# jacobswan1/ViTCAP

Hardware: AMD Instinct MI355X
Metric: images/sec end-to-end greedy caption (20 tok), ViT-B/16-384 (higher is better)
Workload: dtype bf16; 1 GPU; BASELINE configs[1]: ViT-B/16-384 greedy decode (20 tok), batch 64 bf16 per GPU, seeded random-init weights, uniform(-1,1) 384x384 images resident in HBM; batch_per_gpu=64, global_batch=64, decode=greedy, max_length=20, parallelism=replicas x1 (no data-path collective), launch=2-slot batch pipeline (encode of step i+1 || decode of step i), eager launches, streams_per_gpu=2

## Files before the change

vitcap_amd/csrc/call_state.h:

```cpp
#pragma once
#include <hip/hip_runtime.h>
#include <stdint.h>

void vitcap_set_error(const char* fmt, ...);

extern thread_local const int32_t* vc_tls_live;
struct VcEosExtra { int32_t id[3]; };
extern thread_local VcEosExtra vc_tls_eos_extra;
extern thread_local bool vc_tls_walk_rev;
extern thread_local bool vc_tls_zigzag;
extern thread_local const uint32_t* vc_tls_drop_salt;
extern thread_local hipEvent_t vc_tls_kev_start, vc_tls_kev_stop;
extern thread_local bool vc_tls_kev_used;
```

vitcap_amd/csrc/decode.hip:

```cpp
#include "common.h"
#include "rng.h"

namespace {

struct ArgMax {
  float v;
  int i;
};
__device__ __forceinline__ ArgMax am_better(ArgMax a, ArgMax b) {
  return (b.v > a.v || (b.v == a.v && b.i < a.i)) ? b : a;
}
__device__ __forceinline__ ArgMax wave_argmax(ArgMax a) {
#pragma unroll
  for (int o = 32; o > 0; o >>= 1) {
    ArgMax b;
    b.v = __shfl_xor(a.v, o, 64);
    b.i = __shfl_xor(a.i, o, 64);
    a = am_better(a, b);
  }
  return a;
}

__global__ void greedy_init_kernel(int64_t* ids, int32_t* unf, float* sum_lp, float* cnt, int B, int max_len, int bos,
                                   int pad, int32_t* live) {
// ... 307 lines not shown
  if (lane == 0) { s_am[w] = best; s_second[w] = second; s_f[w] = bx; }
  __syncthreads();
  if (tid == 0) {
    ArgMax bb = s_am[0];
    float ss = s_second[0], xx = s_f[0];
    for (int k = 1; k < 16; ++k) {
      const ArgMax nb = am_better(bb, s_am[k]);
      ss = fmaxf(fmaxf(ss, s_second[k]), (nb.i == bb.i) ? s_am[k].v : bb.v);
      xx = (nb.i == bb.i) ? xx : s_f[k];
      bb = nb;
    }
    if (margin_out) margin_out[(size_t)b * max_len + t] = bb.v - ss;
    const float lp = xx - m - logf(z);
    const int u = unf[b];
    const int add = u ? bb.i : pad;
    float s = sum_lp[b] + lp * (float)u;
    float c = cnt[b] + (float)u;
    int nu = u * (vc_is_eos(add, eos, eos_x) ? 0 : 1);
    int64_t outtok = add;
    if (t == max_len - 1) {
      if (raw_last) raw_last[b] = add;
      if (nu) outtok = eos;
      logprob_out[b] = s / c;
    }
    ids[(size_t)b * max_len + t] = outtok;
    sum_lp[b] = s;
    cnt[b] = c;
    unf[b] = nu;
    if (live && u && !nu) atomicSub(live, 1);
  }
}

constexpr int TK_PER_THREAD = 32;
__device__ __forceinline__ unsigned long long tk_key(float f, int i);
__device__ __forceinline__ float tk_val(unsigned long long k);
__device__ __forceinline__ int tk_idx(unsigned long long k);
__device__ __forceinline__ unsigned long long wave_max_u64(unsigned long long a);
__global__ __launch_bounds__(1024) void sigmoid_topk_kernel(const float* __restrict__ logits, int ldl, int V, int k,
                                                            float thresh, int64_t* __restrict__ out_ids,
                                                            float* __restrict__ out_prob,
                                                            int64_t* __restrict__ out_len) {
  __shared__ unsigned long long s_wmax[2][16];
  const int b = blockIdx.x, tid = threadIdx.x, lane = tid & 63, w = tid >> 6;
  const float* row = logits + (size_t)b * ldl;
  unsigned long long key[TK_PER_THREAD];
  unsigned long long tmax = 0ull;
#pragma unroll
  for (int j = 0; j < TK_PER_THREAD; ++j) {
    const int i = tid + j * 1024;
    key[j] = i < V ? tk_key(1.0f / (1.0f + expf(-row[i])), i) : 0ull;
    tmax = key[j] > tmax ? key[j] : tmax;
  }
  int nlen = 0;
  for (int r = 0; r < k; ++r) {
    const unsigned long long wm = wave_max_u64(tmax);
    if (lane == 0) s_wmax[r & 1][w] = wm;
    __syncthreads();
    unsigned long long best = s_wmax[r & 1][0];
#pragma unroll
    for (int q = 1; q < 16; ++q) {
      const unsigned long long c = s_wmax[r & 1][q];
      best = c > best ? c : best;
    }
    if (tid == 0) {
      const float pv = tk_val(best);
      out_ids[(size_t)b * k + r] = tk_idx(best);
      out_prob[(size_t)b * k + r] = pv;
      if (pv >= thresh) ++nlen;
    }
    if (tmax == best) {
      tmax = 0ull;
#pragma unroll
      for (int j = 0; j < TK_PER_THREAD; ++j) {
        if (key[j] == best) key[j] = 0ull;
        tmax = key[j] > tmax ? key[j] : tmax;
      }
    }
  }
  if (tid == 0) out_len[b] = nlen;
}


__device__ __forceinline__ unsigned long long tk_key(float f, int i) {
  unsigned u = __float_as_uint(f);
  u = (u & 0x80000000u) ? ~u : (u | 0x80000000u);
  return ((unsigned long long)u << 32) | (unsigned)(~i);
}
__device__ __forceinline__ float tk_val(unsigned long long k) {
  unsigned u = (unsigned)(k >> 32);
  u = (u & 0x80000000u) ? (u & 0x7fffffffu) : ~u;
  return __uint_as_float(u);
}
__device__ __forceinline__ int tk_idx(unsigned long long k) { return (int)(~(unsigned)k); }
__device__ __forceinline__ unsigned long long wave_max_u64(unsigned long long a) {
#pragma unroll
  for (int o = 32; o > 0; o >>= 1) {
    const unsigned lo = __shfl_xor((unsigned)a, o, 64), hi = __shfl_xor((unsigned)(a >> 32), o, 64);
    const unsigned long long b = ((unsigned long long)hi << 32) | lo;
    a = b > a ? b : a;
  }
  return a;
}

__global__ __launch_bounds__(1024) void row_topk_lse_kernel(const float* __restrict__ logits, int ldl, int V, int k,
                                                            float* __restrict__ out_val, int* __restrict__ out_idx,
                                                            float* __restrict__ out_lse, const int32_t* __restrict__ live) {
  VC_LIVE_EXIT(live);
  constexpr int CAP = TK_PER_THREAD * 16;
  __shared__ unsigned long long s_cand[16][16];
  __shared__ unsigned long long s_list[CAP];
  __shared__ unsigned long long s_thr;
  __shared__ float s_sum[16];
// ... 400 lines not shown
  VC_REQUIRE(logits && ids && rows > 0 && V > 0 && ldl >= V && t >= 1 && t <= ld_ids && t <= 64 && penalty > 0.f,
             "repetition_penalty: bad arguments (t=%d, penalty=%g)", t, (double)penalty);
  hipLaunchKernelGGL(repetition_penalty_kernel, dim3((rows + 3) / 4), dim3(256), 0, (hipStream_t)stream, logits, ldl, V, ids,
                     ld_ids, t, penalty, rows, vc_tls_live);
  VC_LAUNCH_CHECK("repetition_penalty");
  return VITCAP_OK;
}

extern "C" int vitcap_greedy_init(int64_t* ids, int32_t* unfinished, float* sum_lp, float* cnt, int B, int max_len,
                                  int bos, int pad, void* stream) {
  VC_REQUIRE(ids && unfinished && sum_lp && cnt && B > 0 && max_len > 1, "greedy_init: bad arguments");
  const int n = B * max_len;
  hipLaunchKernelGGL(greedy_init_kernel, dim3((n + 255) / 256), dim3(256), 0, (hipStream_t)stream, ids, unfinished,
                     sum_lp, cnt, B, max_len, bos, pad, (int32_t*)vc_tls_live);
  VC_LAUNCH_CHECK("greedy_init");
  return VITCAP_OK;
}

extern "C" int vitcap_greedy_step(const float* logits, int ldl, int V, int64_t* ids, int32_t* unfinished,
                                  float* sum_lp, float* cnt, float* logprob_out, float* margin_out, int64_t* raw_last,
                                  int B, int t, int max_len, int eos, int pad, void* stream) {
  VC_REQUIRE(logits && ids && unfinished && sum_lp && cnt && logprob_out, "greedy_step: null pointer");
  VC_REQUIRE(B > 0 && V > 0 && ldl >= V && t >= 1 && t < max_len, "greedy_step: bad sizes (t=%d)", t);
  hipLaunchKernelGGL(greedy_step_kernel, dim3(B), dim3(1024), 0, (hipStream_t)stream, logits, ldl, V, ids, unfinished,
                     sum_lp, cnt, logprob_out, margin_out, raw_last, t, max_len, eos, pad, (int32_t*)vc_tls_live, vc_tls_eos_extra);
  VC_LAUNCH_CHECK("greedy_step");
  return VITCAP_OK;
}

extern "C" int vitcap_sigmoid_topk(const float* logits, int ldl, int V, int k, float thresh, int64_t* out_ids,
                                   float* out_prob, int64_t* out_len, int B, void* stream) {
  VC_REQUIRE(logits && out_ids && out_prob && out_len && B > 0, "sigmoid_topk: bad arguments");
  VC_REQUIRE(k >= 1 && k <= 64 && V <= TK_PER_THREAD * 1024 && ldl >= V, "sigmoid_topk: k=%d V=%d unsupported", k, V);
  hipLaunchKernelGGL(sigmoid_topk_kernel, dim3(B), dim3(1024), 0, (hipStream_t)stream, logits, ldl, V, k, thresh,
                     out_ids, out_prob, out_len);
  VC_LAUNCH_CHECK("sigmoid_topk");
  return VITCAP_OK;
}


extern "C" int vitcap_row_topk_lse(const float* logits, int ldl, int V, int k, float* out_val, int32_t* out_idx,
                                   float* out_lse, int rows, void* stream) {
  VC_REQUIRE(logits && out_val && out_idx && out_lse && rows > 0, "row_topk_lse: bad arguments");
  VC_REQUIRE(k >= 1 && k <= 16 && V <= TK_PER_THREAD * 1024 && ldl >= V, "row_topk_lse: k=%d V=%d unsupported", k, V);
  hipLaunchKernelGGL(row_topk_lse_kernel, dim3(rows), dim3(1024), 0, (hipStream_t)stream, logits, ldl, V, k, out_val,
                     out_idx, out_lse, vc_tls_live);
  VC_LAUNCH_CHECK("row_topk_lse");
  return VITCAP_OK;
}

extern "C" int vitcap_row_topk_pieces(const float* logits, int ldl, int V, const float* rowstat, int pieces, int k,
                                      float* out_val, int32_t* out_idx, float* out_lse, int rows, void* stream) {
  VC_REQUIRE(logits && rowstat && out_val && out_idx && out_lse && rows > 0, "row_topk_pieces: bad arguments");
  VC_REQUIRE(k >= 1 && k <= 16 && ldl >= V && pieces >= k && pieces <= 1024 && pieces * 32 >= V,
             "row_topk_pieces: k=%d V=%d pieces=%d unsupported", k, V, pieces);
  hipLaunchKernelGGL(row_topk_pieces_kernel, dim3(rows), dim3(256), 0, (hipStream_t)stream, logits, ldl, V, rowstat, pieces, k,
                     out_val, out_idx, out_lse, vc_tls_live);
  VC_LAUNCH_CHECK("row_topk_pieces");
  return VITCAP_OK;
}

static BeamState make_state(const vitcap_beam_state* s) {
  BeamState st;
  st.ids_in = s->ids_in; st.ids_out = s->ids_out; st.beam_scores = s->beam_scores; st.parent = s->parent;
  st.done = s->done; st.has_hyp = s->has_hyp; st.hyp_score = s->hyp_score; st.hyp_len = s->hyp_len;
  st.hyp_tok = s->hyp_tok;
  st.n_keep = s->n_keep;
  return st;
// ... 97 lines not shown
```

vitcap_amd/csrc/engine.cpp:

```cpp
#include <stdlib.h>
#include <string.h>

#include <new>
#include <utility>

#include "engine_internal.h"
#include "engine_layout.h"

using namespace vc;

namespace {

vitcap_gen_opts default_opts() {
  vitcap_gen_opts o;
  memset(&o, 0, sizeof(o));
  o.abi = VITCAP_ABI_VERSION;
  o.num_beams = 1;
  o.seqs_per_image = 1;
  o.num_keep_best = 1;
  o.max_length = VITCAP_MAXLEN;
  o.bos_token_id = 101; o.eos_token_id = 102; o.pad_token_id = 0; o.mask_token_id = 103;
  o.length_penalty = 1.0f;
  o.repetition_penalty = 1.0f;
  o.sampling.do_sample = 0; o.sampling.temperature = 1.0f; o.sampling.top_k = 0; o.sampling.top_p = 1.0f; o.sampling.seed = 0u;
// ... 50 lines not shown
    OPT_REQ(o.tag_visible == 0, "gen_opts: use_cbs with tag tokens visible to the caption is not built");
    OPT_REQ(o.max_length >= 3, "gen_opts: use_cbs needs max_length >= 3 (got %d)", o.max_length);
    OPT_REQ(o.cbs_no_repeat == 0 || o.cbs_no_repeat == 1, "gen_opts: cbs_no_repeat must be 0 or 1 (got %d)", o.cbs_no_repeat);
    for (int i = 0; i < 16; ++i)
      OPT_REQ(o.cbs_bad_ending[i] >= -1 && o.cbs_bad_ending[i] < VITCAP_VOCAB, "gen_opts: cbs_bad_ending[%d] = %d is neither -1 nor a token id", i, o.cbs_bad_ending[i]);
  }
#undef OPT_REQ
  return VITCAP_OK;
}

#define CK(call)             \
  do {                       \
    int rc_ = (call);        \
    if (rc_ != 0) return rc_; \
  } while (0)

#define HIPCK(call, what)                                                              \
  do {                                                                                 \
    hipError_t he_ = (call);                                                           \
    if (he_ != hipSuccess) {                                                           \
      vitcap_set_error("%s: %s", what, hipGetErrorString(he_));                        \
      return VITCAP_ELAUNCH;                                                           \
    }                                                                                  \
  } while (0)

void drop_graphs(vitcap_engine* e) {
  for (auto& g : e->graphs) {
    (void)hipGraphExecDestroy(g.exec);
    (void)hipGraphDestroy(g.graph);
  }
  e->graphs.clear();
}

enum { ROLE_SIDE = 0, ROLE_DEC2 = 1, ROLE_PART0 = 2 , ROLE_COUNT = 5 };
hipStream_t role_stream(int role) {
  static std::mutex mu;
  static hipStream_t pool[64][ROLE_COUNT] = {};
  int dev = 0;
  if (hipGetDevice(&dev) != hipSuccess || dev < 0 || dev >= 64 || role < 0 || role >= ROLE_COUNT) return nullptr;
  std::lock_guard<std::mutex> lk(mu);
  if (!pool[dev][role] && hipStreamCreateWithFlags(&pool[dev][role], hipStreamNonBlocking) != hipSuccess) pool[dev][role] = nullptr;
  return pool[dev][role];
}

int ensure_lane(int role, hipStream_t& st, hipEvent_t& ev_fork, hipEvent_t& ev_join, const char* what) {
  if (st) return VITCAP_OK;
  hipStream_t rs = role_stream(role);
  if (!rs || (!ev_fork && hipEventCreateWithFlags(&ev_fork, hipEventDisableTiming) != hipSuccess) ||
      (!ev_join && hipEventCreateWithFlags(&ev_join, hipEventDisableTiming) != hipSuccess)) {
    vitcap_set_error("%s stream creation failed", what);
    return VITCAP_ELAUNCH;
  }
  st = rs;
  return VITCAP_OK;
}
int ev_record(hipEvent_t ev, void* s, const char* what, const char* edge) {
  const hipError_t he = hipEventRecord(ev, (hipStream_t)s);
  if (he != hipSuccess) { vitcap_set_error("%s %s record: %s", what, edge, hipGetErrorString(he)); return VITCAP_ELAUNCH; }
  return VITCAP_OK;
}
int ev_wait(void* s, hipEvent_t ev, const char* what, const char* edge) {
  const hipError_t he = hipStreamWaitEvent((hipStream_t)s, ev, 0);
  if (he != hipSuccess) { vitcap_set_error("%s %s wait: %s", what, edge, hipGetErrorString(he)); return VITCAP_ELAUNCH; }
  return VITCAP_OK;
}
int fork(void* from, void* to, hipEvent_t ev, const char* what) {
  CK(ev_record(ev, from, what, "fork"));
// ... 119 lines not shown
                const vitcap_vit_block_w* next = nullptr) const {
    const int M = B * NV;
    if (!have_ln1) { CK(vitcap_layernorm_fwd(x_in, D, bw.n1_g, bw.n1_b, 1e-6f, h, nullptr, M, D, s)); zz(); }
    CK(gemm(h, D, bw.qkv_w, bw.qkv_b, nullptr, 0, qkv, 3 * D, M, 3 * D, D, VITCAP_ACT_NONE, VITCAP_OUT_BF16));
    zz();
    CK(vitcap_attn_dense_fwd(qkv, h, B, NV, 0.125f, s));
    zz();
    CK(gemm_ln(h, D, bw.proj_w, bw.proj_b, x_in, x, M, D, bw.n2_g, bw.n2_b, 1e-6f, h, nullptr));
    CK(gemm(h, D, bw.fc1_w, bw.fc1_b, nullptr, 0, mlp, 4 * D, M, 4 * D, D, VITCAP_ACT_GELU_ERF, VITCAP_OUT_BF16));
    zz();
    if (next) {
      CK(gemm_ln(mlp, 4 * D, bw.fc2_w, bw.fc2_b, x, x, M, 4 * D, next->n1_g, next->n1_b, 1e-6f, h, nullptr));
    } else {
      CK(gemm(mlp, 4 * D, bw.fc2_w, bw.fc2_b, x, D, x, D, M, D, 4 * D, VITCAP_ACT_NONE, VITCAP_OUT_F32));
      zz();
    }
    return VITCAP_OK;
  }

  int vit_block_cls_only(const vitcap_vit_block_w& bw, float* x, void* h, void* qkv, void* mlp, void* cls_h) const {
    const int M = B * NV;
    const int RS = NV * D;
    CK(gemm(h, D, (const char*)bw.qkv_w + (size_t)D * D * 2, bw.qkv_b + D, nullptr, 0, (char*)qkv + (size_t)D * 2, 3 * D, M, 2 * D, D,
            VITCAP_ACT_NONE, VITCAP_OUT_BF16));
    CK(gemm(h, RS, bw.qkv_w, bw.qkv_b, nullptr, 0, qkv, NV * 3 * D, B, D, D, VITCAP_ACT_NONE, VITCAP_OUT_BF16));
    CK(vitcap_attn_dense_fwd_rows(qkv, h, B, NV, 1, 0.125f, s));
    CK(gemm(h, RS, bw.proj_w, bw.proj_b, x, RS, x, RS, B, D, D, VITCAP_ACT_NONE, VITCAP_OUT_F32));
    CK(vitcap_layernorm_fwd(x, RS, bw.n2_g, bw.n2_b, 1e-6f, cls_h, nullptr, B, D, s));
    CK(gemm(cls_h, D, bw.fc1_w, bw.fc1_b, nullptr, 0, mlp, 4 * D, B, 4 * D, D, VITCAP_ACT_GELU_ERF, VITCAP_OUT_BF16));
    CK(gemm(mlp, 4 * D, bw.fc2_w, bw.fc2_b, x, RS, x, RS, B, D, 4 * D, VITCAP_ACT_NONE, VITCAP_OUT_F32));
    return VITCAP_OK;
  }

  int tag_branch() const {
    float* xt = p<float>(lo.xt);
    const float* xf = p<float>(lo.x);
    for (int i = 0; i < 3; ++i)
      CK(vit_block(w.tag_blocks[i], i == 0 ? xf : xt, xt, ws + lo.th, ws + lo.tqkv, ws + lo.tmlp, i > 0, &w.tag_blocks[i + 1]));
    if (e->full_last_tag_block)
      CK(vit_block(w.tag_blocks[3], xt, xt, ws + lo.th, ws + lo.tqkv, ws + lo.tmlp, true, nullptr));
    else
      CK(vit_block_cls_only(w.tag_blocks[3], xt, ws + lo.th, ws + lo.tqkv, ws + lo.tmlp, ws + lo.pool_in));
    CK(vitcap_gather_rows_bf16(xt, NV, ws + lo.pool_in, B, D, s));
    CK(gemm(ws + lo.pool_in, D, w.pooler_w, w.pooler_b, nullptr, 0, ws + lo.pooled, D, B, D, D, VITCAP_ACT_TANH, VITCAP_OUT_BF16));
    CK(gemm(ws + lo.pooled, D, w.tag_logit.dense_w, w.tag_logit.dense_b, nullptr, 0, ws + lo.tg_f, D, B, D, D, VITCAP_ACT_GELU_ERF,
            VITCAP_OUT_F32));
    CK(vitcap_layernorm_fwd(p<float>(lo.tg_f), D, w.tag_logit.ln_g, w.tag_logit.ln_b, 1e-12f, ws + lo.tg_b, nullptr, B, D, s));
    CK(gemm(ws + lo.tg_b, D, w.tag_logit.dec_w, w.tag_logit.dec_b, nullptr, 0, ws + lo.tag_logits, VP, B, VP, D, VITCAP_ACT_NONE,
            VITCAP_OUT_F32));
    CK(vitcap_sigmoid_topk(p<float>(lo.tag_logits), VP, VITCAP_VOCAB, TOPK, 0.2f, p<int64_t>(lo.tag_ids), p<float>(lo.tag_prob),
                           p<int64_t>(lo.tag_len), B, s));
    return VITCAP_OK;
  }

  int encode_part(const void* image, int image_is_bf16, bool allow_fork) const {
    float* x = p<float>(lo.x);
    CK(vitcap_patch_gather(image, image_is_bf16, ws + lo.patches, B, s));
    vitcap_gemm_desc d = desc(B * 576, D, D, D, D, VITCAP_ACT_NONE, VITCAP_OUT_F32);
    d.ldr = D;
    d.row_group = 576; d.out_group_rows = NV; d.out_row_off = 1; d.res_periodic = 1;
    CK(gemm_desc(ws + lo.patches, w.patch_w, w.patch_b, w.pos_embed + D, x, d));
    zz();
    CK(vitcap_cls_rows(w.cls_token, w.pos_embed, x, B, NV, s));
    const bool forked = allow_fork && o.gemm_mode == VITCAP_GEMM_TILES && B <= 128;
    float* x2 = p<float>(lo.x2);
    for (int i = 0; i < 12; ++i) {
      if (i == 8 && forked) {
        CK(ensure_lane(ROLE_SIDE, e->side, e->ev_fork, e->ev_join, "encode: side"));
        CK(fork(s, e->side, e->ev_fork, "encode:"));
        CK(on(e->side).tag_branch());
        CK(ev_record(e->ev_join, e->side, "encode:", "join"));
      }
      const vitcap_vit_block_w* next = i + 1 < 12 ? &w.blocks[i + 1] : nullptr;
      if (i < 8) CK(vit_block(w.blocks[i], x, x, ws + lo.h, ws + lo.qkv, ws + lo.mlp, i > 0, next));
      else CK(vit_block(w.blocks[i], i == 8 ? x : x2, x2, ws + lo.h, ws + lo.qkv, ws + lo.mlp, true, next));
    }
    if (forked) return ev_wait(s, e->ev_join, "encode:", "join");
    return tag_branch();
  }

  int prefill_tags() const {
    const int n = lo.NT, R = B * n, S2 = SV + n;
    if (!o.tagemb_cls && !(w.xword_emb && w.xpos_emb && w.xtype_emb && w.xemb_ln_g && w.xemb_ln_b)) {
      vitcap_set_error("prefill: tag_visible with tagemb != 'cls' needs bert.extra_embeddings bound (vitcap_weights.x*)");
      return VITCAP_ESTATE;
    }
    for (int v = 0; v < 2; ++v)
      CK(vitcap_tag_embed(p<int64_t>(lo.tag_ids), n, o.tag_pos0, v == 0, o.tagemb_cls, w.cls.dec_w, w.word_emb, w.pos_emb, w.type_emb,
                          w.emb_ln_g, w.emb_ln_b, w.xword_emb, w.xpos_emb, w.xtype_emb, w.xemb_ln_g, w.xemb_ln_b, 1e-12f,
                          p<float>(lo.tagx_f(v)), p(lo.tagx_b(v)), B, s));
    for (int l = 0; l < 4; ++l) {
      const vitcap_bert_layer_w& lw = w.dec[l];
      if (l < 3)
        CK(vitcap_copy_row_blocks(ws + lo.dqkv[l], SV, 0, 3 * D, D, ws + lo.jqkv, JROWS, 0, 3 * D, D, SV, 2 * D, B, s));
      for (int v = 0; v < 2; ++v) {
        char* tq = p(lo.tqkv_c(v, l));
        float* xf = p<float>(lo.tagx_f(v));
        char* xb = p(lo.tagx_b(v));
        if (l == 3) {
          CK(gemm(xb, D, (const char*)lw.qkv_w + (size_t)D * D * 2, lw.qkv_b + D, nullptr, 0, tq + (size_t)D * 2, 3 * D, R, 2 * D, D,
                  VITCAP_ACT_NONE, VITCAP_OUT_BF16));
          continue;
        }
        CK(gemm(xb, D, lw.qkv_w, lw.qkv_b, nullptr, 0, tq, 3 * D, R, 3 * D, D, VITCAP_ACT_NONE, VITCAP_OUT_BF16));
        CK(vitcap_copy_row_blocks(tq, n, 0, 3 * D, 0, ws + lo.jqkv, JROWS, SV, 3 * D, 0, n, 3 * D, B, s));
        CK(vitcap_attn_dense_fwd_train_rows(ws + lo.jqkv, ws + lo.jout, p<float>(lo.jlse), B, S2, JROWS, 0.125f, 0.f, 0u, 0, 0, 512, S2, s));
        CK(vitcap_copy_row_blocks(ws + lo.jout, JROWS, SV, D, 0, ws + lo.tg_ctx, n, 0, D, 0, n, D, B, s));
        CK(gemm(ws + lo.tg_ctx, D, lw.ao_w, lw.ao_b, xf, D, ws + lo.tg_tmp, D, R, D, D, VITCAP_ACT_NONE, VITCAP_OUT_F32));
        CK(vitcap_layernorm_fwd(p<float>(lo.tg_tmp), D, lw.ao_g, lw.ao_beta, 1e-12f, ws + lo.tg_sa_b, p<float>(lo.tg_sa_f), R, D, s));
        CK(gemm(ws + lo.tg_sa_b, D, lw.i_w, lw.i_b, nullptr, 0, ws + lo.tg_mlp, 4 * D, R, 4 * D, D, VITCAP_ACT_GELU_ERF, VITCAP_OUT_BF16));
        CK(gemm(ws + lo.tg_mlp, 4 * D, lw.o_w, lw.o_b, p<float>(lo.tg_sa_f), D, ws + lo.tg_tmp, D, R, D, 4 * D, VITCAP_ACT_NONE,
// ... 24 lines not shown
      CK(vitcap_attn_dense_fwd(dq, ws + lo.h, B, SV, 0.125f, s));
      zz();
      CK(gemm_ln(ws + lo.h, D, lw.ao_w, lw.ao_b, vis_f, ws + lo.dtmp, M, D, lw.ao_g, lw.ao_beta, 1e-12f, ws + lo.da_b, p<float>(lo.da_f)));
      CK(gemm(ws + lo.da_b, D, lw.i_w, lw.i_b, nullptr, 0, ws + lo.mlp, 4 * D, M, 4 * D, D, VITCAP_ACT_GELU_ERF, VITCAP_OUT_BF16));
      zz();
      CK(gemm_ln(ws + lo.mlp, 4 * D, lw.o_w, lw.o_b, p<float>(lo.da_f), ws + lo.dtmp, M, 4 * D, lw.o_g, lw.o_beta, 1e-12f, vis_b, vis_f));
    }
    if (lo.NT > 0) CK(prefill_tags());
    return VITCAP_OK;
  }

  int encode_parts() const {
    static const int env = [] { const char* v = getenv("VITCAP_ENCODE_SPLIT"); return v ? atoi(v) : -1; }();
    int np = env >= 0 ? env : o.encode_parts;
    if (np == 0) np = (o.gemm_mode == VITCAP_GEMM_TILES && B >= 32) ? 2 : 1;
    if (np > 4) np = 4;
    if (B < 8 || lo.NT > 0) np = 1;
    return np;
  }

  int encode(const void* image, int image_is_bf16) const {
    if (!image) { vitcap_set_error("encode: null image"); return VITCAP_EINVAL; }
    if (e->timing) e->timing_this_step = (e->timing_seen++ % e->timing_stride) == 0;
    const int np = encode_parts();
    if (np < 2) return encode_part(image, image_is_bf16, true);
    for (int i = 0; i < np - 1; ++i) CK(ensure_lane(ROLE_PART0 + i, e->part[i], e->ev_pfork, e->ev_pjoin[i], "encode: part"));
    CK(ev_record(e->ev_pfork, s, "encode: split", "fork"));
    const size_t img_bytes = (size_t)3 * 384 * 384 * (image_is_bf16 ? 2 : 4);
    int i0[5];
    for (int i = 0; i <= np; ++i) i0[i] = (int)((long long)B * i / np);
    Layout lv[4];
    for (int i = 0; i < np; ++i) lv[i] = lo.from_image(i0[i]);
    auto part = [&](int i) { return view(lv[i], i0[i + 1] - i0[i], i == 0 ? s : (void*)e->part[i - 1]); };
    for (int i = 0; i < np; ++i) {
      if (i > 0) CK(ev_wait(part(i).s, e->ev_pfork, "encode: split", "fork"));
      CK(part(i).encode_part((const char*)image + (size_t)i0[i] * img_bytes, image_is_bf16, false));
    }
    for (int i = 0; i < np; ++i) {
      CK(part(i).prefill_part());
      if (i > 0) CK(join(part(i).s, s, e->ev_pjoin[i - 1], "encode: split"));
    }
    return VITCAP_OK;
  }

  int prefill() const {
    if (encode_parts() >= 2) return VITCAP_OK;
    return prefill_part();
  }

  int step_forward(int t, const int64_t* ids_all, char* tcache, bool embed, bool rowstat, const Part& pt) const {
    const int NS = lo.NS, K = lo.K, L = lo.L;
    const int ns = pt.ns, R = 2 * ns;
    const size_t s0 = (size_t)pt.s0, i0 = (size_t)pt.i0;
    float* xs_f = p<float>(lo.xs_f, s0);
    char* xs_b = p(lo.xs_b, s0);
    char* sqkv = p(lo.sqkv, s0);
    char* sctx = p(lo.sctx, s0);
    float* sa_f = p<float>(lo.sa_f, s0);
    char* sa_b = p(lo.sa_b, s0);
    char* smlp = p(lo.smlp, s0);
    char* hd_b = p(lo.hd_b, s0);
    float* slab = p<float>(lo.spart, s0);
    if (embed)
      CK(vitcap_embed_step(ids_all + s0 * L, L, t, o.mask_token_id, w.word_emb, w.pos_emb, w.type_emb, w.emb_ln_g, w.emb_ln_b, 1e-12f,
                           xs_f, xs_b, ns, s));
    const bool small = 2 * NS <= 1024;
    auto proj = [&](const void* A, const void* W, const float* bias, void* C, int N, int act) {
      return small ? gemm_ring(A, D, W, bias, C, N, R, N, D, act, VITCAP_OUT_BF16)
                   : gemm(A, D, W, bias, nullptr, 0, C, N, R, N, D, act, VITCAP_OUT_BF16);
    };
    auto slabs = [&](const void* A, int lda, const void* W, int M, int Kd, int& split) {
      if (!small) return gemm_split(A, lda, W, slab, M, D, Kd, split);
      split = Kd / D;
      return gemm_ring(A, lda, W, nullptr, slab, D, M, D, Kd, VITCAP_ACT_NONE, VITCAP_OUT_F32);
// ... 238 lines not shown
  if (tag_topk_out)
    HIPCK(hipMemcpyAsync(tag_topk_out, ws + lo.tag_ids, B * lo.tag_ids.unit, hipMemcpyDeviceToDevice, (hipStream_t)s), "tags: topk copy");
  return VITCAP_OK;
}

}

extern "C" void vitcap_gen_opts_init(vitcap_gen_opts* o) {
  if (o) *o = default_opts();
}
extern "C" int vitcap_gen_opts_check(const vitcap_gen_opts* o) {
  if (!o) return VITCAP_OK;
  return check_opts(*o);
}

extern "C" int vitcap_engine_create(vitcap_engine** out) {
  if (!out) return VITCAP_EINVAL;
  *out = new (std::nothrow) vitcap_engine();
  if (*out) {
    const char* t = getenv("VITCAP_FULL_TAG_BLOCK");
    (*out)->full_last_tag_block = t ? atoi(t) != 0 : false;
  }
  return *out ? VITCAP_OK : VITCAP_EINVAL;
}

extern "C" void vitcap_engine_destroy(vitcap_engine* e) {
  if (!e) return;
  for (auto& t : e->pool) {
    (void)hipEventDestroy(t.start);
    (void)hipEventDestroy(t.stop);
  }
  drop_graphs(e);
  if (e->cap) (void)hipStreamDestroy(e->cap);
  for (hipEvent_t ev : {e->ev_fork, e->ev_join, e->ev_dfork, e->ev_djoin, e->ev_pjoin[0], e->ev_pjoin[1], e->ev_pjoin[2], e->ev_pfork})
    if (ev) (void)hipEventDestroy(ev);
  delete e;
}
extern "C" int vitcap_engine_graph_count(vitcap_engine* e) { return e ? (int)e->graphs.size() : 0; }

extern "C" int vitcap_engine_bind_weights(vitcap_engine* e, const vitcap_weights* w) {
  if (!e || !w) { vitcap_set_error("bind_weights: null"); return VITCAP_EINVAL; }
  const void* const* p = (const void* const*)w;
  const size_t required = offsetof(vitcap_weights, xword_emb) / sizeof(void*);
  for (size_t i = 0; i < required; ++i)
    if (!p[i]) { vitcap_set_error("bind_weights: pointer #%zu of vitcap_weights is NULL", i); return VITCAP_EINVAL; }
  std::lock_guard<std::mutex> lk(e->mu);
  e->w = *w;
  e->bound = true;
  drop_graphs(e);
  return VITCAP_OK;
}

extern "C" size_t vitcap_engine_workspace_bytes(int B, const vitcap_gen_opts* opts) {
  const vitcap_gen_opts o = opts_or_default(opts);
  if (B <= 0 || check_opts(o) != VITCAP_OK) return 0;
  return Layout(B, o).off;
}

extern "C" int vitcap_engine_encode(vitcap_engine* e, const void* image, int image_is_bf16, int B, const vitcap_gen_opts* opts,
                                    void* workspace, size_t workspace_bytes, void* s) {
  const vitcap_gen_opts o = opts_or_default(opts);
  Layout lo;
  CK(enter(e, B, o, workspace, workspace_bytes, lo));
  std::lock_guard<std::mutex> lk(e->mu);
  return Enq(e, B, o, lo, (char*)workspace, s, Enq::ENCODE).encode(image, image_is_bf16);
}

// ... 15 lines not shown
  return decode_locked(e, B, o, lo, (char*)workspace, out_ids, out_logprobs, out_last_tok, s);
}

extern "C" int vitcap_engine_tags(vitcap_engine* e, int B, const vitcap_gen_opts* opts, void* workspace, float* tag_logits_out,
                                  int64_t* tag_topk_out, void* s) {
  const vitcap_gen_opts o = opts_or_default(opts);
  if (!e || B <= 0 || !workspace || check_opts(o) != VITCAP_OK) { vitcap_set_error("tags: bad arguments"); return VITCAP_EINVAL; }
  return tags_copy(Layout(B, o), B, (char*)workspace, tag_logits_out, tag_topk_out, s);
}

extern "C" int vitcap_engine_generate(vitcap_engine* e, const void* image, int image_is_bf16, int B, const vitcap_gen_opts* opts,
                                      void* workspace, size_t workspace_bytes, int64_t* out_ids, float* out_logprobs,
                                      float* tag_logits_out, int64_t* tag_topk_out, void* s) {
  const vitcap_gen_opts o = opts_or_default(opts);
  Layout lo;
  CK(enter(e, B, o, workspace, workspace_bytes, lo));
  char* ws = (char*)workspace;
  std::lock_guard<std::mutex> lk(e->mu);
  CK(Enq(e, B, o, lo, ws, s, Enq::ENCODE).encode(image, image_is_bf16));
  CK(Enq(e, B, o, lo, ws, s, Enq::ENCODE).prefill());
  CK(decode_locked(e, B, o, lo, ws, out_ids, out_logprobs, nullptr, s));
  return tags_copy(lo, B, ws, tag_logits_out, tag_topk_out, s);
}

extern "C" const void* vitcap_engine_tap(vitcap_engine* e, const char* name, void* workspace, int B, const vitcap_gen_opts* opts) {
  const vitcap_gen_opts o = opts_or_default(opts);
  if (!e || !name || !workspace || B <= 0 || check_opts(o) != VITCAP_OK) return nullptr;
  const Layout lo(B, o);
  char* ws = (char*)workspace;
  if (!strcmp(name, "last_token")) return ws + lo.last_tok;
  if (!strcmp(name, "hidden")) return ws + lo.x2;
  if (!strcmp(name, "tag_hidden")) return ws + lo.xt;
  if (!strcmp(name, "vis")) return ws + lo.vis_f;
  if (!strcmp(name, "logits_last")) return ws + lo.logits;
  if (!strcmp(name, "margins")) return ws + lo.margins;
  if (!strcmp(name, "tag_logits")) return ws + lo.tag_logits;
  if (!strcmp(name, "tag_prob")) return ws + lo.tag_prob;
  if (!strcmp(name, "tag_len")) return ws + lo.tag_len;
  if (!strcmp(name, "ids")) return ws + lo.ids;
  if (!strcmp(name, "live")) return ws + lo.live;
  if (!strcmp(name, "cbs_npred")) return lo.cbs ? ws + lo.cbs_npred : nullptr;
  return nullptr;
}
```

vitcap_amd/csrc/engine_internal.h:

```cpp
#pragma once
#include <hip/hip_runtime.h>

#include <mutex>
#include <vector>

#include "../../include/vitcap_hip.h"
#include "call_state.h"

struct GemmTiming {
  hipEvent_t start, stop;
  hipEvent_t kstart, kstop;
  bool kernel_bound;
  int variant;
  double flops;
};

struct GraphEntry {
  int B;
  void* ws;
  vitcap_gen_opts opts;
  hipGraph_t graph;
  hipGraphExec_t exec;
};

struct vitcap_engine {
  vitcap_weights w;
  bool bound = false;
  bool timing = false;
  int timing_stride = 1;
  long long timing_seen = 0;
  bool timing_this_step = true;
  std::mutex mu;
  hipStream_t side = nullptr;
  hipStream_t cap = nullptr;
  hipEvent_t ev_fork = nullptr, ev_join = nullptr;
  hipStream_t dec2 = nullptr;
  hipEvent_t ev_dfork = nullptr, ev_djoin = nullptr;
  hipStream_t part[3] = {nullptr, nullptr, nullptr};
  hipEvent_t ev_pfork = nullptr, ev_pjoin[3] = {nullptr, nullptr, nullptr};
  bool full_last_tag_block = false;
  std::vector<GemmTiming> pool;
  size_t used = 0;
  std::vector<GraphEntry> graphs;
};
```

vitcap_amd/csrc/engine_layout.h:

```cpp
#pragma once
#include "../../include/vitcap_hip.h"

namespace vc __attribute__((visibility("hidden"))) {

constexpr int D = VITCAP_HID;
constexpr int NV = VITCAP_NVIS;
constexpr int SV = VITCAP_NVIS + 1;
constexpr int VP = VITCAP_VOCAB_PAD;
constexpr int TOPK = 50;
constexpr int JROWS = 640;
constexpr int SPLIT_AO = 6, SPLIT_FC2 = 12, SPLIT_MAX = 12;
constexpr int RS_PIECES = 2 * (VP / 64);
constexpr size_t VT_BYTES = (size_t)12 * 64 * 608 * 2;

enum Scope { IMG, SEQ, FIXED };

struct Buf {
  size_t off = 0;
  size_t unit = 0;
  Scope scope = FIXED;
  operator size_t() const { return off; }
  template <class T = char>
  T* at(char* ws, size_t i = 0) const { return (T*)(ws + off + i * unit); }
};

#define VC_WS_BUFFERS(X, XA)                                                                                                       \
  X(patches, IMG, 576 * D * 2, true)                                                                                               \
  X(x, IMG, NV * D * 4, true)                                                                                                      \
  X(x2, IMG, NV * D * 4, true)              \
  X(xt, IMG, NV * D * 4, true)                                                                                                     \
  X(h, IMG, SV * D * 2, true)                                                                                                      \
  X(qkv, IMG, NV * 3 * D * 2, true)                                                                                                \
  X(mlp, IMG, SV * 4 * D * 2, true)                                                                                                \
  X(th, IMG, NV * D * 2, true)                             \
  X(tqkv, IMG, NV * 3 * D * 2, true)                                                                                               \
  X(tmlp, IMG, NV * 4 * D * 2, true)                                                                                               \
  X(vis_f, IMG, SV * D * 4, true)                                                                                                  \
  X(vis_b, IMG, SV * D * 2, true)                                                                                                  \
  XA(dqkv, 4, IMG, SV * 3 * D * 2, true)                                                                                           \
  X(da_f, IMG, SV * D * 4, true)                                                                                                   \
  X(da_b, IMG, SV * D * 2, true)                                                                                                   \
  X(dtmp, IMG, SV * D * 4, true)                                                                                                   \
  X(pool_in, IMG, D * 2, true)                                                                                                     \
  X(pooled, IMG, D * 2, true)                                                                                                      \
  X(tg_f, IMG, D * 4, true)                                                                                                        \
  X(tg_b, IMG, D * 2, true)                                                                                                        \
  X(tag_logits, IMG, VP * 4, true)                                                                                                 \
  X(tag_ids, IMG, TOPK * 8, true)                                                                                                  \
  X(tag_prob, IMG, TOPK * 4, true)                                                                                                 \
  X(tag_len, IMG, 8, true)                                                                                                         \
                                                                      \
  X(xs_f, SEQ, 2 * D * 4, true)                                                                                                    \
  X(xs_b, SEQ, 2 * D * 2, true)                                                                                                    \
  X(sqkv, SEQ, 2 * 3 * D * 2, true)                                                                                                \
  X(sctx, SEQ, 2 * D * 2, true)                                                                                                    \
  X(spart, SEQ, SPLIT_MAX * 2 * D * 4, true)                                   \
  X(sa_f, SEQ, 2 * D * 4, true)                                                                                                    \
  X(sa_b, SEQ, 2 * D * 2, true)                                                                                                    \
  X(smlp, SEQ, 2 * 4 * D * 2, true)                                                                                                \
  X(tcache, SEQ, 4 * L * 2 * D * 2, true)                                      \
  X(tcache2, SEQ, 4 * L * 2 * D * 2, two)                                                                                          \
  X(hd_f, SEQ, D * 4, true)                                                                                                        \
  X(hd_b, SEQ, D * 2, true)                                                                                                        \
  X(logits, SEQ, VP * 4, true)                                                                                                     \
  X(rowstat, SEQ, RS_PIECES * 16, true)                                                                                            \
  X(ids, SEQ, L * 8, true)                                                                                                         \
  X(ids2, SEQ, L * 8, two)                                                                                                         \
  X(unf, SEQ, 4, true)                                                                                                             \
  X(sum_lp, SEQ, 4, true)                                                                                                          \
  X(cnt, SEQ, 4, true)                                                                                                             \
  X(margins, SEQ, L * 4, true)                                                                                                     \
  X(logprob, SEQ, 4, true)                                                                                                         \
  X(last_tok, SEQ, 8, true)                                                                                                        \
  X(live, FIXED, 256, true)                                                                                                        \
    \
                                                                                         \
  X(tagx_f_a, IMG, NT * D * 4, NT > 0)                                                                                             \
  X(tagx_b_a, IMG, NT * D * 2, NT > 0)                                                                                             \
  XA(tqkv_c_a, 4, IMG, NT * 3 * D * 2, NT > 0)                                                                                     \
  X(tagx_f_b, IMG, NT * D * 4, NT > 0)                                                                                             \
  X(tagx_b_b, IMG, NT * D * 2, NT > 0)                                                                                             \
  XA(tqkv_c_b, 4, IMG, NT * 3 * D * 2, NT > 0)                                                                                     \
  X(jqkv, IMG, JROWS * 3 * D * 2, NT > 0)                 \
// ... 98 lines not shown
```

vitcap_amd/csrc/error.cpp:

```cpp
#include <hip/hip_runtime.h>
#include <stdarg.h>
#include <stdio.h>
#include <stdint.h>
#include "../../include/vitcap_hip.h"
#include "call_state.h"

static thread_local char g_err[512] = "";
thread_local const int32_t* vc_tls_live = nullptr;
thread_local VcEosExtra vc_tls_eos_extra = {{-1, -1, -1}};
thread_local hipEvent_t vc_tls_kev_start = nullptr, vc_tls_kev_stop = nullptr;
thread_local bool vc_tls_kev_used = false;
thread_local bool vc_tls_walk_rev = false;
thread_local bool vc_tls_zigzag = false;
thread_local const uint32_t* vc_tls_drop_salt = nullptr;
extern "C" int vitcap_set_dropout_salt(const void* device_u32) {
  vc_tls_drop_salt = (const uint32_t*)device_u32;
  return 0;
}

void vitcap_set_error(const char* fmt, ...) {
  va_list ap;
  va_start(ap, fmt);
  vsnprintf(g_err, sizeof(g_err), fmt, ap);
  va_end(ap);
}

extern "C" const char* vitcap_last_error(void) { return g_err; }
extern "C" int vitcap_version(void) { return VITCAP_ABI_VERSION; }
```

Before: 4026 images/sec.

## Split tag top-k into per-wave select and merge, optionally offload tag head

Replaces the block-wide iterative top-k, which needs a block barrier per selected element, with per-wave local top-k lists merged by a single wave. When scratch is provided, it runs as a two-kernel select/merge that spreads each row over more blocks. An opt-in env variable can also fork the tag head (pooler, tag logits, top-k) onto side streams to overlap with prefill. This adds scratch memory and extra launches, and the side-stream path stays off by default.

Measured after the change: 4032 images/sec (median of 4 runs). About the same (+0.1%).

```diff
diff --git a/vitcap_amd/csrc/call_state.h b/vitcap_amd/csrc/call_state.h
--- a/vitcap_amd/csrc/call_state.h
+++ b/vitcap_amd/csrc/call_state.h
@@ -12,3 +12,5 @@
 extern thread_local const uint32_t* vc_tls_drop_salt;
 extern thread_local hipEvent_t vc_tls_kev_start, vc_tls_kev_stop;
 extern thread_local bool vc_tls_kev_used;
+constexpr int VC_TOPK_LISTS = 32, VC_TOPK_SLOTS = 64;
+extern thread_local unsigned long long* vc_tls_topk_scratch;
diff --git a/vitcap_amd/csrc/decode.hip b/vitcap_amd/csrc/decode.hip
--- a/vitcap_amd/csrc/decode.hip
+++ b/vitcap_amd/csrc/decode.hip
@@ -363,52 +363,94 @@
 }
 
 constexpr int TK_PER_THREAD = 32;
+constexpr int TK_LISTS = VC_TOPK_LISTS, TK_SLOTS = VC_TOPK_SLOTS;
 __device__ __forceinline__ unsigned long long tk_key(float f, int i);
 __device__ __forceinline__ float tk_val(unsigned long long k);
 __device__ __forceinline__ int tk_idx(unsigned long long k);
 __device__ __forceinline__ unsigned long long wave_max_u64(unsigned long long a);
+
+template <int KPL>
+__device__ __forceinline__ void tk_load_chunk(const float* __restrict__ row, int V, int c0, int ch, int lane,
+                                              unsigned long long (&key)[KPL]) {
+#pragma unroll
+  for (int j = 0; j < KPL; ++j) {
+    const int o = lane + j * 64, i = c0 + o;
+    key[j] = (o < ch && i < V) ? tk_key(1.0f / (1.0f + expf(-row[i])), i) : 0ull;
+  }
+}
+template <int KPL>
+__device__ __forceinline__ void tk_wave_select(unsigned long long (&key)[KPL], int k, int lane, unsigned long long* list) {
+  unsigned long long tmax = 0ull, mine = 0ull;
+#pragma unroll
+  for (int j = 0; j < KPL; ++j) tmax = key[j] > tmax ? key[j] : tmax;
+  for (int r = 0; r < k; ++r) {
+    const unsigned long long best = wave_max_u64(tmax);
+    if (lane == r) mine = best;
+    if (tmax == best && best != 0ull) {
+      tmax = 0ull;
+#pragma unroll
+      for (int j = 0; j < KPL; ++j) {
+        if (key[j] == best) key[j] = 0ull;
+        tmax = key[j] > tmax ? key[j] : tmax;
+      }
+    }
+  }
+  if (lane < k) list[lane] = mine;
+}
+__device__ __forceinline__ void tk_wave_merge(const unsigned long long* lists, int nl, int k, float thresh, int lane,
+                                              int64_t* __restrict__ ids, float* __restrict__ prob, int64_t* __restrict__ len) {
+  const unsigned long long* mylist = lists + (lane < nl ? lane : 0) * TK_SLOTS;
+  int pos = 0;
+  unsigned long long head = lane < nl ? mylist[0] : 0ull, mine = 0ull;
+  for (int r = 0; r < k; ++r) {
+    const unsigned long long best = wave_max_u64(head);
+    if (lane == r) mine = best;
+    if (head == best && best != 0ull) {
+      ++pos;
+      head = pos < k ? mylist[pos] : 0ull;
+    }
+  }
+  const float pv = tk_val(mine);
+  if (lane < k) {
+    ids[lane] = tk_idx(mine);
+    prob[lane] = pv;
+  }
+  const unsigned long long over = __ballot(lane < k && pv >= thresh);
+  if (lane == 0) *len = __popcll(over);
+}
+
 __global__ __launch_bounds__(1024) void sigmoid_topk_kernel(const float* __restrict__ logits, int ldl, int V, int k,
                                                             float thresh, int64_t* __restrict__ out_ids,
                                                             float* __restrict__ out_prob,
                                                             int64_t* __restrict__ out_len) {
-  __shared__ unsigned long long s_wmax[2][16];
+  __shared__ unsigned long long s_list[16 * TK_SLOTS];
   const int b = blockIdx.x, tid = threadIdx.x, lane = tid & 63, w = tid >> 6;
-  const float* row = logits + (size_t)b * ldl;
+  const int ch = (V + 15) / 16;
   unsigned long long key[TK_PER_THREAD];
-  unsigned long long tmax = 0ull;
-#pragma unroll
-  for (int j = 0; j < TK_PER_THREAD; ++j) {
-    const int i = tid + j * 1024;
-    key[j] = i < V ? tk_key(1.0f / (1.0f + expf(-row[i])), i) : 0ull;
-    tmax = key[j] > tmax ? key[j] : tmax;
-  }
-  int nlen = 0;
-  for (int r = 0; r < k; ++r) {
-    const unsigned long long wm = wave_max_u64(tmax);
-    if (lane == 0) s_wmax[r & 1][w] = wm;
-    __syncthreads();
-    unsigned long long best = s_wmax[r & 1][0];
-#pragma unroll
-    for (int q = 1; q < 16; ++q) {
-      const unsigned long long c = s_wmax[r & 1][q];
-      best = c > best ? c : best;
-    }
-    if (tid == 0) {
-      const float pv = tk_val(best);
-      out_ids[(size_t)b * k + r] = tk_idx(best);
-      out_prob[(size_t)b * k + r] = pv;
-      if (pv >= thresh) ++nlen;
-    }
-    if (tmax == best) {
-      tmax = 0ull;
-#pragma unroll
-      for (int j = 0; j < TK_PER_THREAD; ++j) {
-        if (key[j] == best) key[j] = 0ull;
-        tmax = key[j] > tmax ? key[j] : tmax;
-      }
-    }
-  }
-  if (tid == 0) out_len[b] = nlen;
+  tk_load_chunk<TK_PER_THREAD>(logits + (size_t)b * ldl, V, w * ch, ch, lane, key);
+  tk_wave_select<TK_PER_THREAD>(key, k, lane, s_list + w * TK_SLOTS);
+  __syncthreads();
+  if (w == 0) tk_wave_merge(s_list, 16, k, thresh, lane, out_ids + (size_t)b * k, out_prob + (size_t)b * k, out_len + b);
+}
+
+__global__ __launch_bounds__(256) void sigmoid_topk_select_kernel(const float* __restrict__ logits, int ldl, int V, int k,
+                                                                  unsigned long long* __restrict__ scratch) {
+  const int b = blockIdx.y, lane = threadIdx.x & 63, c = blockIdx.x * 4 + (threadIdx.x >> 6);
+  const int ch = (V + TK_LISTS - 1) / TK_LISTS;
+  unsigned long long key[16];
+  tk_load_chunk<16>(logits + (size_t)b * ldl, V, c * ch, ch, lane, key);
+  tk_wave_select<16>(key, k, lane, scratch + ((size_t)b * TK_LISTS + c) * TK_SLOTS);
+}
+__global__ __launch_bounds__(64) void sigmoid_topk_merge_kernel(const unsigned long long* __restrict__ scratch, int k, float thresh,
+                                                                int64_t* __restrict__ out_ids, float* __restrict__ out_prob,
+                                                                int64_t* __restrict__ out_len) {
+  __shared__ unsigned long long s_list[TK_LISTS * TK_SLOTS];
+  const int b = blockIdx.x, lane = threadIdx.x;
+  const unsigned long long* src = scratch + (size_t)b * TK_LISTS * TK_SLOTS;
+  for (int l = 0; l < TK_LISTS; ++l)
+    if (lane < k) s_list[l * TK_SLOTS + lane] = src[l * TK_SLOTS + lane];
+  __syncthreads();
+  tk_wave_merge(s_list, TK_LISTS, k, thresh, lane, out_ids + (size_t)b * k, out_prob + (size_t)b * k, out_len + b);
 }
 
 
@@ -875,8 +917,14 @@
                                    float* out_prob, int64_t* out_len, int B, void* stream) {
   VC_REQUIRE(logits && out_ids && out_prob && out_len && B > 0, "sigmoid_topk: bad arguments");
   VC_REQUIRE(k >= 1 && k <= 64 && V <= TK_PER_THREAD * 1024 && ldl >= V, "sigmoid_topk: k=%d V=%d unsupported", k, V);
-  hipLaunchKernelGGL(sigmoid_topk_kernel, dim3(B), dim3(1024), 0, (hipStream_t)stream, logits, ldl, V, k, thresh,
-                     out_ids, out_prob, out_len);
+  if (unsigned long long* scratch = vc_tls_topk_scratch) {
+    hipLaunchKernelGGL(sigmoid_topk_select_kernel, dim3(TK_LISTS / 4, B), dim3(256), 0, (hipStream_t)stream, logits, ldl, V, k, scratch);
+    hipLaunchKernelGGL(sigmoid_topk_merge_kernel, dim3(B), dim3(64), 0, (hipStream_t)stream, scratch, k, thresh, out_ids, out_prob,
+                       out_len);
+  } else {
+    hipLaunchKernelGGL(sigmoid_topk_kernel, dim3(B), dim3(1024), 0, (hipStream_t)stream, logits, ldl, V, k, thresh,
+                       out_ids, out_prob, out_len);
+  }
   VC_LAUNCH_CHECK("sigmoid_topk");
   return VITCAP_OK;
 }
diff --git a/vitcap_amd/csrc/engine.cpp b/vitcap_amd/csrc/engine.cpp
--- a/vitcap_amd/csrc/engine.cpp
+++ b/vitcap_amd/csrc/engine.cpp
@@ -106,7 +106,7 @@
   e->graphs.clear();
 }
 
-enum { ROLE_SIDE = 0, ROLE_DEC2 = 1, ROLE_PART0 = 2 , ROLE_COUNT = 5 };
+enum { ROLE_SIDE = 0, ROLE_DEC2 = 1, ROLE_PART0 = 2 , ROLE_TAG0 = 5 , ROLE_COUNT = 9 };
 hipStream_t role_stream(int role) {
   static std::mutex mu;
   static hipStream_t pool[64][ROLE_COUNT] = {};
@@ -292,28 +292,37 @@
     return VITCAP_OK;
   }
 
-  int tag_branch() const {
+  int tag_blocks() const {
     float* xt = p<float>(lo.xt);
     const float* xf = p<float>(lo.x);
     for (int i = 0; i < 3; ++i)
       CK(vit_block(w.tag_blocks[i], i == 0 ? xf : xt, xt, ws + lo.th, ws + lo.tqkv, ws + lo.tmlp, i > 0, &w.tag_blocks[i + 1]));
     if (e->full_last_tag_block)
-      CK(vit_block(w.tag_blocks[3], xt, xt, ws + lo.th, ws + lo.tqkv, ws + lo.tmlp, true, nullptr));
-    else
-      CK(vit_block_cls_only(w.tag_blocks[3], xt, ws + lo.th, ws + lo.tqkv, ws + lo.tmlp, ws + lo.pool_in));
-    CK(vitcap_gather_rows_bf16(xt, NV, ws + lo.pool_in, B, D, s));
+      return vit_block(w.tag_blocks[3], xt, xt, ws + lo.th, ws + lo.tqkv, ws + lo.tmlp, true, nullptr);
+    return vit_block_cls_only(w.tag_blocks[3], xt, ws + lo.th, ws + lo.tqkv, ws + lo.tmlp, ws + lo.pool_in);
+  }
+
+  int tag_head() const {
+    CK(vitcap_gather_rows_bf16(p<float>(lo.xt), NV, ws + lo.pool_in, B, D, s));
     CK(gemm(ws + lo.pool_in, D, w.pooler_w, w.pooler_b, nullptr, 0, ws + lo.pooled, D, B, D, D, VITCAP_ACT_TANH, VITCAP_OUT_BF16));
     CK(gemm(ws + lo.pooled, D, w.tag_logit.dense_w, w.tag_logit.dense_b, nullptr, 0, ws + lo.tg_f, D, B, D, D, VITCAP_ACT_GELU_ERF,
             VITCAP_OUT_F32));
     CK(vitcap_layernorm_fwd(p<float>(lo.tg_f), D, w.tag_logit.ln_g, w.tag_logit.ln_b, 1e-12f, ws + lo.tg_b, nullptr, B, D, s));
     CK(gemm(ws + lo.tg_b, D, w.tag_logit.dec_w, w.tag_logit.dec_b, nullptr, 0, ws + lo.tag_logits, VP, B, VP, D, VITCAP_ACT_NONE,
             VITCAP_OUT_F32));
-    CK(vitcap_sigmoid_topk(p<float>(lo.tag_logits), VP, VITCAP_VOCAB, TOPK, 0.2f, p<int64_t>(lo.tag_ids), p<float>(lo.tag_prob),
-                           p<int64_t>(lo.tag_len), B, s));
-    return VITCAP_OK;
-  }
-
-  int encode_part(const void* image, int image_is_bf16, bool allow_fork) const {
+    vc_tls_topk_scratch = p<unsigned long long>(lo.tag_scr);
+    const int rc = vitcap_sigmoid_topk(p<float>(lo.tag_logits), VP, VITCAP_VOCAB, TOPK, 0.2f, p<int64_t>(lo.tag_ids), p<float>(lo.tag_prob),
+                                       p<int64_t>(lo.tag_len), B, s);
+    vc_tls_topk_scratch = nullptr;
+    return rc;
+  }
+
+  int tag_branch() const {
+    CK(tag_blocks());
+    return tag_head();
+  }
+
+  int encode_part(const void* image, int image_is_bf16, bool allow_fork, int tag_lane = -1) const {
     float* x = p<float>(lo.x);
     CK(vitcap_patch_gather(image, image_is_bf16, ws + lo.patches, B, s));
     vitcap_gemm_desc d = desc(B * 576, D, D, D, D, VITCAP_ACT_NONE, VITCAP_OUT_F32);
@@ -336,7 +345,11 @@
       else CK(vit_block(w.blocks[i], i == 8 ? x : x2, x2, ws + lo.h, ws + lo.qkv, ws + lo.mlp, true, next));
     }
     if (forked) return ev_wait(s, e->ev_join, "encode:", "join");
-    return tag_branch();
+    if (tag_lane < 0) return tag_branch();
+    CK(tag_blocks());
+    CK(fork(s, e->tlane[tag_lane], e->ev_tfork[tag_lane], "encode: tag head"));
+    CK(on(e->tlane[tag_lane]).tag_head());
+    return ev_record(e->ev_tjoin[tag_lane], e->tlane[tag_lane], "encode: tag head", "join");
   }
 
   int prefill_tags() const {
@@ -427,14 +440,19 @@
     Layout lv[4];
     for (int i = 0; i < np; ++i) lv[i] = lo.from_image(i0[i]);
     auto part = [&](int i) { return view(lv[i], i0[i + 1] - i0[i], i == 0 ? s : (void*)e->part[i - 1]); };
+    static const int lane_env = [] { const char* v = getenv("VITCAP_TAG_LANE"); return v ? atoi(v) : -1; }();
+    const int lane_mode = lane_env >= 0 && lane_env <= 2 ? lane_env : 0;
+    for (int i = 0; i < np && lane_mode > 0; ++i)
+      CK(ensure_lane(ROLE_TAG0 + (lane_mode == 2 ? i : 0), e->tlane[i], e->ev_tfork[i], e->ev_tjoin[i], "encode: tag head"));
     for (int i = 0; i < np; ++i) {
       if (i > 0) CK(ev_wait(part(i).s, e->ev_pfork, "encode: split", "fork"));
-      CK(part(i).encode_part((const char*)image + (size_t)i0[i] * img_bytes, image_is_bf16, false));
+      CK(part(i).encode_part((const char*)image + (size_t)i0[i] * img_bytes, image_is_bf16, false, lane_mode > 0 ? i : -1));
     }
     for (int i = 0; i < np; ++i) {
       CK(part(i).prefill_part());
       if (i > 0) CK(join(part(i).s, s, e->ev_pjoin[i - 1], "encode: split"));
     }
+    for (int i = 0; i < np && lane_mode > 0; ++i) CK(ev_wait(s, e->ev_tjoin[i], "encode: tag head", "join"));
     return VITCAP_OK;
   }
 
@@ -739,7 +757,9 @@
   }
   drop_graphs(e);
   if (e->cap) (void)hipStreamDestroy(e->cap);
-  for (hipEvent_t ev : {e->ev_fork, e->ev_join, e->ev_dfork, e->ev_djoin, e->ev_pjoin[0], e->ev_pjoin[1], e->ev_pjoin[2], e->ev_pfork})
+  for (hipEvent_t ev : {e->ev_fork, e->ev_join, e->ev_dfork, e->ev_djoin, e->ev_pjoin[0], e->ev_pjoin[1], e->ev_pjoin[2], e->ev_pfork,
+                        e->ev_tfork[0], e->ev_tfork[1], e->ev_tfork[2], e->ev_tfork[3], e->ev_tjoin[0], e->ev_tjoin[1], e->ev_tjoin[2],
+                        e->ev_tjoin[3]})
     if (ev) (void)hipEventDestroy(ev);
   delete e;
 }
@@ -821,6 +841,7 @@
   if (!strcmp(name, "hidden")) return ws + lo.x2;
   if (!strcmp(name, "tag_hidden")) return ws + lo.xt;
   if (!strcmp(name, "vis")) return ws + lo.vis_f;
+  if (!strcmp(name, "vis_b")) return ws + lo.vis_b;
   if (!strcmp(name, "logits_last")) return ws + lo.logits;
   if (!strcmp(name, "margins")) return ws + lo.margins;
   if (!strcmp(name, "tag_logits")) return ws + lo.tag_logits;
diff --git a/vitcap_amd/csrc/engine_internal.h b/vitcap_amd/csrc/engine_internal.h
--- a/vitcap_amd/csrc/engine_internal.h
+++ b/vitcap_amd/csrc/engine_internal.h
@@ -38,6 +38,8 @@
   hipEvent_t ev_dfork = nullptr, ev_djoin = nullptr;
   hipStream_t part[3] = {nullptr, nullptr, nullptr};
   hipEvent_t ev_pfork = nullptr, ev_pjoin[3] = {nullptr, nullptr, nullptr};
+  hipStream_t tlane[4] = {nullptr, nullptr, nullptr, nullptr};
+  hipEvent_t ev_tfork[4] = {nullptr, nullptr, nullptr, nullptr}, ev_tjoin[4] = {nullptr, nullptr, nullptr, nullptr};
   bool full_last_tag_block = false;
   std::vector<GemmTiming> pool;
   size_t used = 0;
diff --git a/vitcap_amd/csrc/engine_layout.h b/vitcap_amd/csrc/engine_layout.h
--- a/vitcap_amd/csrc/engine_layout.h
+++ b/vitcap_amd/csrc/engine_layout.h
@@ -1,5 +1,6 @@
 #pragma once
 #include "../../include/vitcap_hip.h"
+#include "call_state.h"
 
 namespace vc __attribute__((visibility("hidden"))) {
 
@@ -49,6 +50,7 @@
   X(tag_ids, IMG, TOPK * 8, true)                                                                                                  \
   X(tag_prob, IMG, TOPK * 4, true)                                                                                                 \
   X(tag_len, IMG, 8, true)                                                                                                         \
+  X(tag_scr, IMG, VC_TOPK_LISTS * VC_TOPK_SLOTS * 8, true)      \
                                                                       \
   X(xs_f, SEQ, 2 * D * 4, true)                                                                                                    \
   X(xs_b, SEQ, 2 * D * 2, true)                                                                                                    \
diff --git a/vitcap_amd/csrc/error.cpp b/vitcap_amd/csrc/error.cpp
--- a/vitcap_amd/csrc/error.cpp
+++ b/vitcap_amd/csrc/error.cpp
@@ -13,6 +13,7 @@
 thread_local bool vc_tls_walk_rev = false;
 thread_local bool vc_tls_zigzag = false;
 thread_local const uint32_t* vc_tls_drop_salt = nullptr;
+thread_local unsigned long long* vc_tls_topk_scratch = nullptr;
 extern "C" int vitcap_set_dropout_salt(const void* device_u32) {
   vc_tls_drop_salt = (const uint32_t*)device_u32;
   return 0;
```
